# facebookresearch/any4

Measured on AMD Instinct MI355X. Metric: any4 W4A16 GEMM achieved GB/s (m=1, n=k=4096, g=128), higher is better.
Workload: dtype bf16

## Files before the change

any4_amd/csrc/tg_common.cuh:

```cuda
#pragma once
#ifndef GEMV_TRACE
#define GEMV_TRACE 0
#endif
#include <hip/hip_runtime.h>
#include <stdint.h>
#include <stdlib.h>
#include <string.h>
#include <atomic>
#include <type_traits>
#include <utility>

#include "../../include/tinygemm_hip.h"

struct GemmParams {
  const char* x;
  const char* w;
  const char* qinfo;
  const char* lut;
  char* y;
  int32_t m, wrows, k;
  int32_t ntiles;
  int32_t ksuper;
  int32_t gshift;
  int32_t ngroups;
// ... 133 lines not shown
}
inline int pair_b16(int dt, int I, bool qmx, GemmParams& p, int64_t batch, hipStream_t st) {
  return dt == TG_BF16 ? pair_b16_bf16(I, qmx, p, batch, st) : pair_b16_f16(I, qmx, p, batch, st);
}
inline int stream(int dt, bool layout_a, int wpl, bool qmx, const GemmParams& p, int64_t coltiles, int64_t batch, hipStream_t st) {
  return dt == TG_BF16 ? stream_bf16(layout_a, wpl, qmx, p, coltiles, batch, st) : stream_f16(layout_a, wpl, qmx, p, coltiles, batch, st);
}
}

namespace {

typedef __attribute__((ext_vector_type(4))) float f32x4;
typedef __attribute__((ext_vector_type(2))) float f32x2;
typedef __attribute__((ext_vector_type(4))) uint32_t u32x4;
typedef __attribute__((ext_vector_type(2))) uint32_t u32x2;
typedef __attribute__((ext_vector_type(8))) __bf16 bf16x8;
typedef __attribute__((ext_vector_type(2))) __bf16 bf16x2;
typedef __attribute__((ext_vector_type(8))) _Float16 f16x8;
typedef __attribute__((ext_vector_type(2))) _Float16 f16x2;

typedef const __attribute__((address_space(3))) float* lds_cfptr;
typedef __attribute__((address_space(3))) float* lds_fptr;
typedef const __attribute__((address_space(3))) uint16_t* lds_cu16ptr;
typedef const __attribute__((address_space(3))) uint32_t* lds_cu32ptr;
typedef __attribute__((address_space(3))) uint32_t* lds_u32ptr;
typedef const __attribute__((address_space(3))) u32x4* lds_cu32x4ptr;
typedef __attribute__((address_space(3))) u32x4* lds_u32x4ptr;
typedef const __attribute__((address_space(3))) f32x4* lds_cf32x4ptr;
typedef __attribute__((address_space(3))) f32x4* lds_f32x4ptr;

__device__ __forceinline__ float u2f(uint32_t u) { return __builtin_bit_cast(float, u); }
__device__ __forceinline__ uint32_t f2u(float f) { return __builtin_bit_cast(uint32_t, f); }

struct BF16 {
  static __device__ __forceinline__ float to_f32(uint16_t h) { return u2f(((uint32_t)h) << 16); }
  static __device__ __forceinline__ float lo_f32(uint32_t pair) { return u2f(pair << 16); }
  static __device__ __forceinline__ float hi_f32(uint32_t pair) { return u2f(pair & 0xffff0000u); }
  static __device__ __forceinline__ uint32_t pack2(float a, float b) {
    f32x2 v = {a, b};
    return __builtin_bit_cast(uint32_t, __builtin_convertvector(v, bf16x2));
  }
  static __device__ __forceinline__ uint16_t from_f32(float a) { return (uint16_t)(pack2(a, 0.f) & 0xffffu); }
  static __device__ __forceinline__ f32x4 mfma(u32x4 a, u32x4 b, f32x4 c) {
    return __builtin_amdgcn_mfma_f32_16x16x32_bf16(__builtin_bit_cast(bf16x8, a), __builtin_bit_cast(bf16x8, b), c, 0, 0, 0);
  }
};
struct F16 {
  static __device__ __forceinline__ float to_f32(uint16_t h) { return (float)__builtin_bit_cast(_Float16, h); }
  static __device__ __forceinline__ float lo_f32(uint32_t pair) { return to_f32((uint16_t)(pair & 0xffffu)); }
  static __device__ __forceinline__ float hi_f32(uint32_t pair) { return to_f32((uint16_t)(pair >> 16)); }
  static __device__ __forceinline__ uint32_t pack2(float a, float b) {
    f32x2 v = {a, b};
    return __builtin_bit_cast(uint32_t, __builtin_convertvector(v, f16x2));
  }
  static __device__ __forceinline__ uint16_t from_f32(float a) { return (uint16_t)(pack2(a, 0.f) & 0xffffu); }
  static __device__ __forceinline__ f32x4 mfma(u32x4 a, u32x4 b, f32x4 c) {
    return __builtin_amdgcn_mfma_f32_16x16x32_f16(__builtin_bit_cast(f16x8, a), __builtin_bit_cast(f16x8, b), c, 0, 0, 0);
  }
};

__device__ const float kMX4Values[16] = {0.0f,  0.5f,  1.0f,  1.5f,  2.0f,  3.0f,  4.0f,  6.0f,
                                         -0.0f, -0.5f, -1.0f, -1.5f, -2.0f, -3.0f, -4.0f, -6.0f};

template <typename DT>
__device__ __forceinline__ void store_rows4(char* yb, const char* bias, int64_t elem, int rowg, f32x4 acc) {
  u32x2 o = {DT::pack2(acc[0], acc[1]), DT::pack2(acc[2], acc[3])};
  if (bias) {
    const u32x2 bv = *reinterpret_cast<const u32x2*>(bias + (int64_t)rowg * 2);
    o[0] = DT::pack2(DT::lo_f32(o[0]) + DT::lo_f32(bv[0]), DT::hi_f32(o[0]) + DT::hi_f32(bv[0]));
    o[1] = DT::pack2(DT::lo_f32(o[1]) + DT::lo_f32(bv[1]), DT::hi_f32(o[1]) + DT::hi_f32(bv[1]));
  }
  *reinterpret_cast<u32x2*>(yb + elem * 2) = o;
}


__device__ __forceinline__ u32x4 transpose_rows4(u32x4 v) {
  const auto s01 = __builtin_amdgcn_permlane16_swap(v[0], v[1], false, false);
  const auto s23 = __builtin_amdgcn_permlane16_swap(v[2], v[3], false, false);
  const auto t02 = __builtin_amdgcn_permlane32_swap(s01[0], s23[0], false, false);
  const auto t13 = __builtin_amdgcn_permlane32_swap(s01[1], s23[1], false, false);
  return u32x4{t02[0], t13[0], t02[1], t13[1]};
}

struct DeviceScope {
  int prev = -1;
  bool ok = true;
  explicit DeviceScope(int device) {
    if (device < 0) return;
    if (hipGetDevice(&prev) != hipSuccess) { ok = false; return; }
    if (prev != device && hipSetDevice(device) != hipSuccess) ok = false;
    if (prev == device) prev = -1;
  }
  ~DeviceScope() {
    if (prev >= 0) (void)hipSetDevice(prev);
  }
};

inline int launch_status() {
  const hipError_t e = hipGetLastError();
  return e == hipSuccess ? 0 : (int)e;
}

inline bool aligned16(const void* p) { return (reinterpret_cast<uintptr_t>(p) & 15u) == 0; }
inline int64_t cdiv(int64_t a, int64_t b) { return (a + b - 1) / b; }
inline int group_shift(int g) { return g == 32 ? 5 : g == 64 ? 6 : g == 128 ? 7 : 8; }

template <typename D, typename F>
auto assign_if_member(D& d, F f, int) -> decltype(f(d)) { f(d); }
template <typename D, typename F>
void assign_if_member(D&, F, long) {}
template <typename D>
void copy_call(D& d, const GemmParams& p) {
#define TG_COPY(f) assign_if_member(d, [&](auto& t) -> decltype((void)(t.f = p.f)) { t.f = p.f; }, 0)
  TG_COPY(x); TG_COPY(w); TG_COPY(qinfo); TG_COPY(lut); TG_COPY(y);
  TG_COPY(m); TG_COPY(wrows); TG_COPY(k); TG_COPY(ntiles); TG_COPY(ksuper); TG_COPY(gshift); TG_COPY(ngroups); TG_COPY(qtype);
  TG_COPY(stride_x); TG_COPY(stride_w); TG_COPY(stride_qinfo); TG_COPY(stride_lut); TG_COPY(stride_y);
  TG_COPY(bias); TG_COPY(stride_bias); TG_COPY(bias_row_stride);
  TG_COPY(norm_w); TG_COPY(norm_eps); TG_COPY(epilogue); TG_COPY(x_tc); TG_COPY(y_tc); TG_COPY(dry);
#undef TG_COPY
}

template <auto KERN>
int prepare_lds_kernel() {
  static std::atomic<uint64_t> done{0};
  int dev = 0;
  if (hipGetDevice(&dev) != hipSuccess) return TG_E_DEVICE;
  if (dev >= 0 && dev < 64 && ((done.load(std::memory_order_relaxed) >> dev) & 1u)) return 0;
  hipFuncAttributes fa;
  hipError_t e = hipFuncGetAttributes(&fa, reinterpret_cast<const void*>(KERN));
  if (e != hipSuccess) return (int)e;
  if (fa.sharedSizeBytes != 0) return TG_E_INTERNAL;
  e = hipFuncSetAttribute(reinterpret_cast<const void*>(KERN), hipFuncAttributeMaxDynamicSharedMemorySize, 160 * 1024);
  if (e != hipSuccess) return (int)e;
  if (dev >= 0 && dev < 64) done.fetch_or(1ull << dev, std::memory_order_relaxed);
  return 0;
}


inline int cu_count() {
  static std::atomic<int> cache[64];
  int dev = 0;
  if (hipGetDevice(&dev) != hipSuccess || dev < 0 || dev >= 64) return 256;
  int v = cache[dev].load(std::memory_order_relaxed);
  if (v > 0) return v;
  if (hipDeviceGetAttribute(&v, hipDeviceAttributeMultiprocessorCount, dev) != hipSuccess || v <= 0) v = 256;
  cache[dev].store(v, std::memory_order_relaxed);
  return v;
}


#if !defined(TG_DEV) && !defined(TG_DEV_MIN)
#if defined(TG_PAIR_R) || defined(TG_PAIR_ABL) || defined(TG_PAIR_MR1) || defined(TG_PAIR_NSG2) || defined(TG_PAIR_MR1_GPS) || defined(TG_PAIR_RA) ||   \
    defined(TG_PAIR_RA1) || defined(TG_PAIR_RB16) || defined(TG_B16_CHUNK) || defined(TG_PAIR_MIN_ITEMS) || defined(TG_XG_CHUNK) || defined(TG_PAIR_WGS) || \
    defined(TG_PAIR_NSG2_M1) || defined(TG_PAIR_FORCE_XG) || defined(TG_XR_MIN_M) || defined(TG_XR_R) || defined(TG_XR_R8K) || defined(TG_XR_RMX)
#error "the TG_PAIR_* / TG_XG_* / TG_B16_* tuning constants can only be overridden in developer builds (-DTG_DEV or -DTG_DEV_MIN)"
#endif
#endif
#ifndef TG_PAIR_R
#define TG_PAIR_R 2
#endif
#ifndef TG_PAIR_ABL
#define TG_PAIR_ABL 0
#endif
#ifndef TG_PAIR_MR1
#define TG_PAIR_MR1 1
#endif
#ifndef TG_PAIR_NSG2
#define TG_PAIR_NSG2 1
#endif
#ifndef TG_PAIR_NSG2_M1
#define TG_PAIR_NSG2_M1 1
#endif
#ifndef TG_PAIR_MR1_GPS
#define TG_PAIR_MR1_GPS 1
#endif
#ifndef TG_PAIR_RA
#define TG_PAIR_RA 2
#endif
#ifndef TG_PAIR_RA1
#define TG_PAIR_RA1 1
#endif
#ifndef TG_PAIR_RB16
#define TG_PAIR_RB16 2
#endif
#ifndef TG_B16_CHUNK
#define TG_B16_CHUNK 4
#endif
#ifndef TG_TILE_W8_MIN_M
#define TG_TILE_W8_MIN_M 17
#endif
#ifndef TG_TILE_MIN_M_SPLIT
#define TG_TILE_MIN_M_SPLIT 17
#endif
#ifndef TG_TILE_MIN_M
#define TG_TILE_MIN_M 65
#endif
#ifndef TG_M1_DEFAULT_MFMA
#define TG_M1_DEFAULT_MFMA 0
#endif
#ifndef TG_PAIR_MIN_ITEMS
#define TG_PAIR_MIN_ITEMS 192
#endif
#ifndef TG_XG_CHUNK
#define TG_XG_CHUNK 4
#endif
#ifndef TG_XR_MIN_M
#define TG_XR_MIN_M 2
#endif
#ifndef TG_XR_RMX
#define TG_XR_RMX 8
#endif
#ifndef TG_XR_R8K
#define TG_XR_R8K 2
#endif
#ifndef TG_XR_R
#define TG_XR_R 4
#endif
#ifndef TG_PAIR_WGS
#define TG_PAIR_WGS 512
#endif

}
```

any4_amd/csrc/w4_gemm_pair.cuh:

```cuda
#pragma once

__device__ __forceinline__ int64_t tc_a_index(int r, int c, int ctiles) {
  const int t = (r & 7) * 4 + ((c & 7) >> 1);
  const int j = (c & 1) + 2 * ((r >> 3) & 1) + 4 * ((c >> 3) & 1);
  return (((int64_t)(r >> 4) * ctiles + (c >> 4)) * 32 + t) * 8 + j;
}
__device__ __forceinline__ void tc_a_load_chunk(const char* xb, int a, int ch, int ktiles, uint32_t (&d)[16]) {
#pragma unroll
  for (int dw = 0; dw < 16; ++dw) d[dw] = *reinterpret_cast<const uint32_t*>(xb + tc_a_index(a, ch * 32 + 2 * dw, ktiles) * 2);
}

__device__ __forceinline__ u32x4 mx4_cvt_word(uint32_t w, float scale) {
  u32x4 r;
  r[0] = __builtin_bit_cast(uint32_t, __builtin_amdgcn_cvt_scalef32_pk_bf16_fp4(w, scale, 0));
  r[1] = __builtin_bit_cast(uint32_t, __builtin_amdgcn_cvt_scalef32_pk_bf16_fp4(w, scale, 1));
  r[2] = __builtin_bit_cast(uint32_t, __builtin_amdgcn_cvt_scalef32_pk_bf16_fp4(w, scale, 2));
  r[3] = __builtin_bit_cast(uint32_t, __builtin_amdgcn_cvt_scalef32_pk_bf16_fp4(w, scale, 3));
  return r;
}

__device__ __forceinline__ uint32_t mx4_cvt_byte(uint32_t w, float scale, int sel) {
  switch (sel) {
    case 0: return __builtin_bit_cast(uint32_t, __builtin_amdgcn_cvt_scalef32_pk_bf16_fp4(w, scale, 0));
    case 1: return __builtin_bit_cast(uint32_t, __builtin_amdgcn_cvt_scalef32_pk_bf16_fp4(w, scale, 1));
    case 2: return __builtin_bit_cast(uint32_t, __builtin_amdgcn_cvt_scalef32_pk_bf16_fp4(w, scale, 2));
    default: return __builtin_bit_cast(uint32_t, __builtin_amdgcn_cvt_scalef32_pk_bf16_fp4(w, scale, 3));
  }
}

#ifndef TG_PAIR_M1_DOT
#define TG_PAIR_M1_DOT 1
#endif
template <typename DT>
__device__ __forceinline__ float dot2_pair(uint32_t a, uint32_t b, float acc) {
  if constexpr (std::is_same<DT, BF16>::value)
    return __builtin_amdgcn_fdot2_f32_bf16(__builtin_bit_cast(bf16x2, a), __builtin_bit_cast(bf16x2, b), acc, false);
  else
    return __builtin_amdgcn_fdot2(__builtin_bit_cast(f16x2, a), __builtin_bit_cast(f16x2, b), acc, false);
}

struct PairParams {
  const char* x;
  const char* w;
  const char* qinfo;
  const char* lut;
  char* y;
  int32_t m, wrows, k;
  int32_t ntiles;
  int32_t ksuper;
  int32_t gshift;
  int32_t ngroups;
  int32_t qtype;
  int32_t spw;
  int32_t nsg_shift;
  int32_t gch_mask;
  int32_t x_pitch;
  int32_t lds_x;
  int32_t lds_xs;
  int32_t lds_red;
  int32_t rused;
  int32_t xs_rows;
  int32_t red_lanes;
  int32_t red_alias;
  int32_t rblocks;
  int32_t cblocks;
  int32_t items;
  int64_t stride_x, stride_w, stride_qinfo, stride_lut, stride_y;
  const char* bias;
  int64_t stride_bias;
  int64_t bias_row_stride;
  const char* norm_w;
  float norm_eps;
  int32_t epilogue;
  int32_t dry;
  const char* xp;
  const char* xsum;
  int64_t stride_xp, stride_xsum;
  int32_t xw_pitch;
  int32_t xw_bytes;
  int32_t chunk;
  int32_t x_tc, y_tc;
  int32_t y_tiles;
};

typedef __attribute__((ext_vector_type(16))) float f32x16;

template <typename DT>
__device__ __forceinline__ f32x16 mfma32(u32x4 a, u32x4 b, f32x16 c) {
  if constexpr (std::is_same<DT, BF16>::value)
    return __builtin_amdgcn_mfma_f32_32x32x16_bf16(__builtin_bit_cast(bf16x8, a), __builtin_bit_cast(bf16x8, b), c, 0, 0, 0);
  else
    return __builtin_amdgcn_mfma_f32_32x32x16_f16(__builtin_bit_cast(f16x8, a), __builtin_bit_cast(f16x8, b), c, 0, 0, 0);
}

typedef __attribute__((ext_vector_type(4))) float f32x4_t;
template <typename DT>
__device__ __forceinline__ f32x4_t mfma16(u32x4 a, u32x4 b, f32x4_t c) {
  if constexpr (std::is_same<DT, BF16>::value)
    return __builtin_amdgcn_mfma_f32_16x16x32_bf16(__builtin_bit_cast(bf16x8, a), __builtin_bit_cast(bf16x8, b), c, 0, 0, 0);
  else
    return __builtin_amdgcn_mfma_f32_16x16x32_f16(__builtin_bit_cast(f16x8, a), __builtin_bit_cast(f16x8, b), c, 0, 0, 0);
}

__device__ __forceinline__ uint32_t bfi(uint32_t mask, uint32_t a, uint32_t b) {
  uint32_t d;
  asm("v_bfi_b32 %0, %1, %2, %3" : "=v"(d) : "s"(mask), "v"(a), "v"(b));
  return d;
}

template <typename DT>
__device__ __forceinline__ float dot2_ones(uint32_t pair, float acc) {
  if constexpr (std::is_same<DT, BF16>::value)
    return __builtin_amdgcn_fdot2_f32_bf16(__builtin_bit_cast(bf16x2, pair), __builtin_bit_cast(bf16x2, 0x3f803f80u), acc, false);
  else
    return __builtin_amdgcn_fdot2(__builtin_bit_cast(f16x2, pair), __builtin_bit_cast(f16x2, 0x3c003c00u), acc, false);
}

template <typename DT>
__device__ __forceinline__ float chunk_sumsq(const uint32_t (&d)[16]) {
  float s = 0.f;
#pragma unroll
  for (int j = 0; j < 16; ++j) {
    if constexpr (std::is_same<DT, BF16>::value)
      s = __builtin_amdgcn_fdot2_f32_bf16(__builtin_bit_cast(bf16x2, d[j]), __builtin_bit_cast(bf16x2, d[j]), s, false);
    else
      s = __builtin_amdgcn_fdot2(__builtin_bit_cast(f16x2, d[j]), __builtin_bit_cast(f16x2, d[j]), s, false);
  }
  return s;
}
template <typename DT>
__device__ __forceinline__ void chunk_rmsnorm(uint32_t (&d)[16], float rs, const u32x4 (&gw)[4]) {
#pragma unroll
  for (int j = 0; j < 4; ++j) {
    const u32x4 g = gw[j];
#pragma unroll
    for (int e = 0; e < 4; ++e) {
      const uint32_t v = d[4 * j + e];
      const float lo = DT::to_f32(DT::from_f32(DT::lo_f32(v) * rs)) * DT::lo_f32(g[e]);
      const float hi = DT::to_f32(DT::from_f32(DT::hi_f32(v) * rs)) * DT::hi_f32(g[e]);
      d[4 * j + e] = DT::pack2(lo, hi);
    }
  }
}
template <typename DT>
__device__ __forceinline__ uint16_t swiglu16(float gsum, float usum) {
  const float g = DT::to_f32(DT::from_f32(gsum)), u = DT::to_f32(DT::from_f32(usum));
  return DT::from_f32(DT::to_f32(DT::from_f32(g / (1.f + __expf(-g)))) * u);
}

template <typename DT, int I, int GPS, int MR, bool QMX, int R, int NSG = 0, int ABL = 0, bool XG = false, int LAY = 0, bool NORM = false>
__global__ void __launch_bounds__(512, 4) w4_gemm_pair_kernel(const PairParams p) {
  constexpr bool LA = LAY == 1, LB = LAY == 2, T16 = LAY != 0;
  constexpr bool DOT = TG_PAIR_M1_DOT && ABL != 100 && MR == 1 && !T16 && (QMX || NSG > 0);
  constexpr bool MXC = QMX;
  static_assert(!NORM || (!XG && !T16 && !QMX), "fused RMSNorm: the workgroup stages the whole activation block itself");
  constexpr int WAVES = 8;
  constexpr int TILES = 2;
  constexpr int WT = LA ? 1 : TILES;
  constexpr int RW = T16 ? 32 : 32 * TILES;
  static_assert(!T16 || (XG && MR == 4 && (LB || I == 2 || I == 4)), "16x16x32 tiles: workspace activations, one pass of up to 16 rows");
  constexpr int NW = LB ? I / 2 : I;
  using acc_t = typename std::conditional<T16, f32x4_t, f32x16>::type;
  constexpr int CPS = I / 2;
  constexpr int CPG = CPS / GPS;
  constexpr int MREGS = MR == 1 ? 4 : MR;
  constexpr int RF = MR;
  constexpr int MA = T16 ? 16 : 2 * MREGS;
  constexpr int NXW = T16 ? I / 2 : XG ? (MA * 2 * I + 63) / 64 : 1;
  static_assert(!XG || MR <= 4, "XG: one pass is at most 8 activation rows");

  constexpr uint32_t lds0 = 0u;
  const uint32_t lds_x = lds0 + (uint32_t)p.lds_x;
  const uint32_t lds_xs = lds0 + (uint32_t)p.lds_xs;
  const uint32_t lds_red = lds0 + (uint32_t)p.lds_red;

  const int tid = threadIdx.x;
  const int lane = tid & 63;
  const int wave = __builtin_amdgcn_readfirstlane(tid >> 6);
  const int c = lane & 31;
  const int h = lane >> 5;
  const int xa = DOT ? 0 : T16 ? lane & 15 : c;
  const int xq = T16 ? lane >> 4 : 2 * h;
  const int hh = T16 ? lane >> 4 : h;
  auto wrow_local = [&](int t) -> int { return LA ? 16 * ((lane & 15) >> 3) + (lane & 7) + 8 * t : LB ? 16 * t + (lane & 15) : t * 32 + c; };
  const int tcol = tid & 63;
  const int tcol_row = LA ? 16 * ((tcol & 15) >> 3) + (tcol & 7) + 8 * (tcol >> 5) : LB ? 16 * (tcol >> 5) + (tcol & 15) : tcol;

  constexpr bool RR = XG;
  const int chunk = RR ? p.chunk : 1;
  const int it_stride = RR ? (int)gridDim.x * chunk - (chunk - 1) : 1;
  const int it_begin = RR ? (int)blockIdx.x * chunk : (int)(((int64_t)blockIdx.x * p.items) / gridDim.x);
  const int it_end = RR ? p.items : (int)(((int64_t)(blockIdx.x + 1) * p.items) / gridDim.x);
  const int per_problem = p.rblocks * p.cblocks;

  const int s_begin = wave * p.spw;
  const int nl = max(min(p.spw, p.ksuper - s_begin), 0);

  struct Item {
    int b, ct, rb;
  };
  auto decode = [&](int it) -> Item {
    const int b = it / per_problem, r = it - b * per_problem;
    const int ct = r / p.rblocks;
    return Item{b, ct, r - ct * p.rblocks};
  };
  const int adv_b = it_stride / per_problem, adv_r = it_stride - adv_b * per_problem;
  auto advance = [&](const Item& e, bool big) -> Item {
    int b = e.b + (big ? adv_b : 0), r = e.ct * p.rblocks + e.rb + (big ? adv_r : 1);
    if (r >= per_problem) { r -= per_problem; ++b; }
    const int ct = p.cblocks == 1 ? 0 : r / p.rblocks;
    return Item{b, ct, r - ct * p.rblocks};
  };

  uint32_t lp[8];
  auto lut_const = [&]() {
#pragma unroll
    for (int e = 0; e < 16; e += 2) {
      float v0, v1;
      if (p.qtype == TG_Q_INT4) {
        v0 = (float)(e - 8);
        v1 = (float)(e - 7);
      } else {
        const int e1 = e + 1;
        v0 = (e & 8 ? -1.f : 1.f) * ((e & 7) < 5 ? 0.5f * (e & 7) : ((e & 7) == 5 ? 3.f : (e & 7) == 6 ? 4.f : 6.f));
        v1 = (e1 & 8 ? -1.f : 1.f) * ((e1 & 7) < 5 ? 0.5f * (e1 & 7) : ((e1 & 7) == 5 ? 3.f : (e1 & 7) == 6 ? 4.f : 6.f));
      }
      lp[e >> 1] = DT::pack2(v0, v1);
    }
  };
  const bool lut_loaded = p.qtype == TG_Q_ANY4_GLOBAL || p.qtype == TG_Q_ANY4_ROWWISE;
  auto lut_request = [&](const Item& e) {
    const int lrow = min(e.rb * RW + tcol_row, p.wrows - 1);
    const char* lsrc = p.lut + (int64_t)e.b * p.stride_lut + (p.qtype == TG_Q_ANY4_ROWWISE ? (int64_t)lrow * 32 : 0);
    const u32x4 l0 = reinterpret_cast<const u32x4*>(lsrc)[0];
    const u32x4 l1 = reinterpret_cast<const u32x4*>(lsrc)[1];
#pragma unroll
    for (int j = 0; j < 4; ++j) { lp[j] = l0[j]; lp[4 + j] = l1[j]; }
  };

  struct Slot {
    uint32_t w[WT][I];
    uint32_t q[TILES][GPS];
    u32x4 xw[NXW];
  };
  Slot ring[R];
  struct Rows {
    uint32_t wbase[WT];
    uint32_t qrow[TILES];
    uint32_t qrow4[TILES];
    const char* wb;
    const char* qb;
    const char* xpb;
    uint32_t xblk;
    uint32_t xoff[NXW];
  };
  auto rows_of = [&](const Item& e) -> Rows {
    Rows r;
#pragma unroll
    for (int t = 0; t < TILES; ++t) {
      const int row = min(e.rb * RW + wrow_local(t), p.wrows - 1);
      r.qrow[t] = (uint32_t)row;
      r.qrow4[t] = (uint32_t)row * 4u;
      if constexpr (!LA) {
        const int nt = min(row >> 3, p.ntiles - 1);
        r.wbase[t] = ((uint32_t)nt * (uint32_t)p.ksuper * 32u + (uint32_t)(4 * (row & 7) + (LB ? lane >> 4 : 2 * h))) * (uint32_t)(2 * I);
      }
    }
    if constexpr (LA) {
      const int mt = min(e.rb * 2 + ((lane & 15) >> 3), p.ntiles - 1);
      r.wbase[0] = ((uint32_t)mt * (uint32_t)p.ksuper * 32u + (uint32_t)(4 * (lane & 7) + (lane >> 4))) * (uint32_t)(4 * I);
    }
    r.wb = p.w + (int64_t)e.b * p.stride_w;
    r.qb = p.qinfo + (int64_t)e.b * p.stride_qinfo;
    if constexpr (XG) {
      const int rows = min(p.m - e.ct * MA, MA);
      r.xpb = p.xp + (int64_t)e.b * p.stride_xp + (int64_t)e.ct * MA * p.k * 2;
      r.xblk = (uint32_t)(rows * 32 * I);
      if constexpr (T16) {
        r.xblk = (uint32_t)((rows + 1) * 64);
        r.xoff[0] = (uint32_t)(((lane >> 4) * (rows + 1) + min(lane & 15, rows)) * 16);
      } else {
#pragma unroll
        for (int i = 0; i < NXW; ++i) r.xoff[i] = (uint32_t)(lane + 64 * i) * 16u < r.xblk ? (uint32_t)(lane + 64 * i) * 16u : 0u;
      }
    } else {
      r.xpb = nullptr;
      r.xblk = 0;
#pragma unroll
      for (int i = 0; i < NXW; ++i) r.xoff[i] = 0;
    }
    return r;
  };
  auto pin = [](uint32_t& v) -> uint32_t { asm volatile("" : "+v"(v)); return v; };
  auto issue = [&](Rows& rw, int s, Slot& sl, bool valid, bool needq) {
    auto uni = [](uint32_t v) -> uint32_t { return (uint32_t)__builtin_amdgcn_readfirstlane((int)v); };
    const uint32_t sv = valid ? (uint32_t)s : 0u;
    if constexpr (XG) {
#pragma unroll
      for (int i = 0; i < NXW; ++i) {
        if constexpr (T16) {
          if constexpr (ABL == 9 || ABL == 13) sl.xw[i] = u32x4{rw.xoff[0], (uint32_t)s, 0x3f803f80u, 0x3f803f80u};
          else if constexpr (ABL == 12) sl.xw[i] = *reinterpret_cast<const u32x4*>(rw.xpb + uni((uint32_t)i * rw.xblk) + pin(rw.xoff[0]));
          else sl.xw[i] = *reinterpret_cast<const u32x4*>(rw.xpb + uni((sv * CPS + (uint32_t)i) * rw.xblk) + pin(rw.xoff[0]));
          continue;
        }
        if constexpr (ABL == 9) sl.xw[i] = u32x4{rw.xoff[i], (uint32_t)s, 0x3f803f80u, 0x3f803f80u};
// ... 32 lines not shown
      }
    }
  };

  constexpr int EBS = QMX ? 16 / GPS : 1;
  u32x4 ecur[TILES], enext[TILES];
  int eoff_next = 0;
  auto e_request = [&](Rows& rw, int blk, bool valid) {
    const int start = s_begin * GPS + blk * 16;
    const int st = max(min(start & ~3, p.ngroups - 16), 0);
    eoff_next = start - st;
#pragma unroll
    for (int t = 0; t < TILES; ++t)
      enext[t] = *reinterpret_cast<const u32x4*>(rw.qb + (uint32_t)__builtin_amdgcn_readfirstlane(valid ? st : 0) + rw.qrow[t] * (uint32_t)p.ngroups);
  };
  int ebase = 0;
  auto e_dword = [&](int t, int gi) -> uint32_t {
    const int dw = (gi + ebase) >> 2;
    return ecur[t][dw & 3];
  };
  auto e_scale = [&](uint32_t d, int gi) -> float {
    const uint32_t e23 = __builtin_amdgcn_ubfe(d, (uint32_t)(((gi + ebase) & 3) * 8), 8u) << 23;
    const float sc = u2f(e23 > 0x00400000u ? e23 : 0x00400000u);
    return __builtin_fmaf(sc, 0.f, sc);
  };

  const int nch = p.k >> 5;
  auto x_load = [&](const char* xb, int a0, int xi, uint32_t (&d)[16]) {
    const int a = xi / nch, ch = xi - a * nch;
    if (p.x_tc) {
      tc_a_load_chunk(xb, a0 + a, ch, p.k >> 4, d);
      return;
    }
    const u32x4* src = reinterpret_cast<const u32x4*>(xb + ((int64_t)(a0 + a) * p.k + ch * 32) * 2);
#pragma unroll
    for (int j = 0; j < 4; ++j) {
      const u32x4 v = src[j];
      d[4 * j] = v[0]; d[4 * j + 1] = v[1]; d[4 * j + 2] = v[2]; d[4 * j + 3] = v[3];
    }
  };
  auto x_store = [&](int xi, bool on, const uint32_t (&d)[16]) {
    const int a = on ? xi / nch : 0, ch = on ? xi - (xi / nch) * nch : 0;
    if (on) {
      const uint32_t dst = lds_x + (uint32_t)(a * p.x_pitch + ch * 64);
#pragma unroll
      for (int q = 0; q < 4; ++q) {
        u32x4 o;
        o[0] = __builtin_amdgcn_perm(d[q + 4], d[q], 0x05040100u);
        o[1] = __builtin_amdgcn_perm(d[q + 12], d[q + 8], 0x05040100u);
        o[2] = __builtin_amdgcn_perm(d[q + 4], d[q], 0x07060302u);
        o[3] = __builtin_amdgcn_perm(d[q + 12], d[q + 8], 0x07060302u);
        *(lds_u32x4ptr)(dst + (uint32_t)(q * 16)) = o;
      }
    }
    if constexpr (QMX) return;
    float sum = 0.f;
#pragma unroll
    for (int j = 0; j < 16; ++j) sum = dot2_ones<DT>(d[j], sum);
    for (int o = 1; o <= p.gch_mask; o <<= 1) sum += __shfl_xor(sum, o);
    if (on && (ch & p.gch_mask) == 0) *(lds_fptr)(lds_xs + (uint32_t)(((ch >> (p.gshift - 5)) * p.xs_rows + a) * 4)) = sum;
  };
  auto x_stage = [&](int b, int a0, int mrows, bool pre, uint32_t (&xd)[16]) {
    const char* xb = p.x + (int64_t)b * p.stride_x;
    const int xtotal = mrows * nch;
    if constexpr (NORM) {
      const bool on = tid < xtotal;
      if (!pre) {
#pragma unroll
        for (int j = 0; j < 16; ++j) xd[j] = 0u;
        if (on) x_load(xb, a0, tid, xd);
      }
      const int a = on ? tid / nch : 0;
      u32x4 gw[4];
#pragma unroll
      for (int j = 0; j < 4; ++j) gw[j] = reinterpret_cast<const u32x4*>(p.norm_w + (on ? tid - a * nch : 0) * 64)[j];
      float ss = chunk_sumsq<DT>(xd);
      ss = tgl::wave_sum(ss);
      if (lane == 0) *(lds_fptr)(lds_xs + (uint32_t)(wave * 4)) = ss;
      __syncthreads();
      ss = 0.f;
      for (int w0 = a * (nch >> 6); w0 < (a + 1) * (nch >> 6); ++w0) ss += *(lds_fptr)(lds_xs + (uint32_t)(w0 * 4));
      __syncthreads();
      if (on) chunk_rmsnorm<DT>(xd, rsqrtf(ss * (1.0f / (float)p.k) + p.norm_eps), gw);
      pre = true;
    }
    for (int it0 = 0; it0 < xtotal; it0 += 512) {
      const int xi = it0 + tid;
      const bool on = xi < xtotal;
      if (!(pre && it0 == 0)) {
#pragma unroll
        for (int j = 0; j < 16; ++j) xd[j] = 0u;
        if (on) x_load(xb, a0, xi, xd);
      }
      x_store(xi, on, xd);
    }
    if constexpr (!QMX)
      for (int idx = tid; idx < p.ngroups * p.xs_rows; idx += 512)
        if ((idx & (p.xs_rows - 1)) >= mrows) *(lds_fptr)(lds_xs + (uint32_t)(idx * 4)) = 0.f;
    if (tid < CPS * 4) *(lds_u32x4ptr)(lds_x + (uint32_t)(mrows * p.x_pitch + tid * 16)) = u32x4{0, 0, 0, 0};
  };

  constexpr int NXS = T16 ? 2 : 0;
  float xsn[2] = {0.f, 0.f};
  auto xs_request = [&](const Item& e) {
    if constexpr (XG && !QMX) {
      const float* src = reinterpret_cast<const float*>(p.xsum + (int64_t)e.b * p.stride_xsum) + (int64_t)e.ct * p.ngroups * p.xs_rows;
      const int total = p.ngroups * p.xs_rows;
#pragma unroll
      for (int j = 0; j < NXS; ++j) xsn[j] = src[min(tid + 512 * j, total - 1)];
    }
  };
  auto xs_stage = [&](int b, int ct, int mrows) {
    const float* src = reinterpret_cast<const float*>(p.xsum + (int64_t)b * p.stride_xsum) + (int64_t)ct * p.ngroups * p.xs_rows;
    if constexpr (!QMX) {
      const int total = p.ngroups * p.xs_rows;
#pragma unroll
      for (int j = 0; j < NXS; ++j) {
        const int idx = tid + 512 * j;
        if (idx < total) *(lds_fptr)(lds_xs + (uint32_t)(idx * 4)) = (idx & (p.xs_rows - 1)) < mrows ? xsn[j] : 0.f;
      }
      for (int idx = tid + 512 * NXS; idx < total; idx += 512)
        *(lds_fptr)(lds_xs + (uint32_t)(idx * 4)) = (idx & (p.xs_rows - 1)) < mrows ? src[idx] : 0.f;
    }
    if (tid < CPS * 4) *(lds_u32x4ptr)(lds_x + (uint32_t)(WAVES * p.xw_bytes + tid * 16)) = u32x4{0, 0, 0, 0};
  };

  if (it_begin >= it_end) return;
  const Item first = decode(it_begin);
  if (lut_loaded) lut_request(first);
  else lut_const();
  xs_request(first);
  int staged_b = XG ? -1 : first.b, staged_ct = first.ct;
  uint32_t xd0[16];
  if constexpr (!XG) {
    const int mrows0 = min(p.m - first.ct * MA, MA);
#pragma unroll
    for (int j = 0; j < 16; ++j) xd0[j] = 0u;
    if (tid < mrows0 * nch) x_load(p.x + (int64_t)first.b * p.stride_x, first.ct * MA, tid, xd0);
  }
  Rows rcur = rows_of(first);
  if constexpr (QMX) e_request(rcur, 0, nl > 0);
#pragma unroll
  for (int j = 0; j < R; ++j) {
    __builtin_amdgcn_sched_barrier(0);
    issue(rcur, s_begin + j, ring[j], j < nl, NSG == 0 || j % NSG == 0);
  }
  __builtin_amdgcn_sched_barrier(0);
  if constexpr (!XG) x_stage(first.b, first.ct * MA, min(p.m - first.ct * MA, MA), true, xd0);

  uint32_t colreg[TILES];
#pragma unroll
  for (int t = 0; t < TILES; ++t) colreg[t] = (uint32_t)((T16 ? 32 * t + 16 * ((lane >> 4) & 1) + (lane & 15) : t * 32 + c) * 4);

  int table_b = -1;
  Item inext = first;
  int cpos = 0;
  for (int it = it_begin, step = 1; it < it_end; it += step) {
    const bool big = cpos + 1 >= chunk;
    step = big ? it_stride : 1;
    cpos = big ? 0 : cpos + 1;
    const Item cur = inext;
    const int row0 = cur.rb * RW;
    const int a0 = cur.ct * MA;
    const int mrows = min(p.m - a0, MA);
    const bool has_next = it + step < it_end;
    if (has_next) inext = advance(cur, big);
    Rows rnext = rows_of(inext);

    if (!MXC && (it == it_begin || p.qtype == TG_Q_ANY4_ROWWISE || p.red_alias ||
        (p.qtype == TG_Q_ANY4_GLOBAL && cur.b != table_b))) {
      table_b = cur.b;
      uint32_t hw = lp[0];
#pragma unroll
      for (int j = 1; j < 8; ++j) hw = (wave == j) ? lp[j] : hw;
      const uint32_t base = lds0 + (uint32_t)(wave * 2 * 16 * 256 + tcol * 4);
#pragma unroll
      for (int a = 0; a < 16; ++a) {
        const uint32_t e0 = __builtin_amdgcn_perm(hw, lp[a >> 1], (a & 1) ? 0x05040302u : 0x05040100u);
        const uint32_t e1 = __builtin_amdgcn_perm(hw, lp[a >> 1], (a & 1) ? 0x07060302u : 0x07060100u);
        const lds_u32ptr tb = (lds_u32ptr)base;
        tb[a * 64] = e0;
        tb[(16 + a) * 64] = e1;
      }
    }
    if (cur.b != staged_b || cur.ct != staged_ct) {
      staged_b = cur.b;
      staged_ct = cur.ct;
      if constexpr (XG) {
        if (ABL != 11) xs_stage(cur.b, cur.ct, mrows);
      } else {
        uint32_t xd[16];
        x_stage(cur.b, a0, mrows, false, xd);
      }
    }
    if (lut_loaded) lut_request(inext);
    xs_request(inext);
    __syncthreads();

    const bool a_on = xa < mrows;
    const uint32_t xzero = XG ? lds_x + (uint32_t)(WAVES * p.xw_bytes) : lds_x + (uint32_t)(mrows * p.x_pitch);
    const uint32_t xs_mask = 4 * hh < p.xs_rows ? 0xffffffffu : 0u;
    const uint32_t xs_lane = 4 * hh < p.xs_rows ? lds_xs + (uint32_t)(4 * hh * 4) : xzero;
    const uint32_t xwbuf = lds_x + (uint32_t)(wave * p.xw_bytes);
    const uint32_t xrow = !a_on ? xzero : XG ? xwbuf + (uint32_t)(xa * p.xw_pitch + xq * 16) : lds_x + (uint32_t)(xa * p.x_pitch + xq * 16);
    const uint32_t xmask = a_on && !XG ? 0xffffffffu : 0u;
    const uint32_t xw_dst = xwbuf + (uint32_t)((lane / (2 * I)) * p.xw_pitch + (lane % (2 * I)) * 16);

    acc_t acc[TILES];
    float yacc[TILES][RF];
#pragma unroll
    for (int t = 0; t < TILES; ++t) {
#pragma unroll
      for (int r = 0; r < (T16 ? 4 : 16); ++r) acc[t][r] = 0.f;
#pragma unroll
      for (int r = 0; r < RF; ++r) yacc[t][r] = 0.f;
    }
    float gs[TILES], gz[TILES];
    float xsv[RF];
#pragma unroll
    for (int t = 0; t < TILES; ++t) gs[t] = gz[t] = 0.f;
#pragma unroll
    for (int r = 0; r < RF; ++r) xsv[r] = 0.f;

    auto unpack_q = [&](uint32_t q, float& s, float& z) {
      if constexpr (QMX) {
        s = u2f(q == 255u ? 0x7fc00000u : (q == 0u ? 0x00400000u : (q << 23)));
        z = 0.f;
      } else {
        s = DT::lo_f32(q);
        z = DOT && h ? 0.f : DT::hi_f32(q);
      }
    };
    constexpr bool DIFF = MR == 1;
    float dacc[TILES] = {0.f, 0.f};
    float prev[TILES][RF];
#pragma unroll
    for (int t = 0; t < TILES; ++t)
#pragma unroll
      for (int r = 0; r < RF; ++r) prev[t][r] = 0.f;
    auto finalize = [&]() {
#pragma unroll
      for (int t = 0; t < TILES; ++t) {
        if constexpr (DOT) {
          const float d = dacc[t] - prev[t][0];
          prev[t][0] = dacc[t];
          yacc[t][0] = __builtin_fmaf(gz[t], xsv[0], __builtin_fmaf(gs[t], d, yacc[t][0]));
          continue;
        }
        if constexpr (DIFF && RF == 1 && !QMX) {
          float a0 = acc[t][0];
          asm volatile("" : "+v"(a0));
          float d;
          asm("v_sub_f32 %0, %1, %2" : "=v"(d) : "v"(a0), "v"(prev[t][0]));
          prev[t][0] = a0;
          asm("v_fmac_f32 %0, %1, %2" : "+v"(yacc[t][0]) : "v"(gs[t]), "v"(d));
          asm("v_fmac_f32 %0, %1, %2" : "+v"(yacc[t][0]) : "v"(gz[t]), "v"(xsv[0]));
          asm volatile("" : "+v"(acc[t]));
          asm volatile("" ::"v"(acc[t][1]), "v"(acc[t][2]), "v"(acc[t][3]));
          continue;
        }
#pragma unroll
        for (int r = 0; r < RF; ++r) {
          float d = acc[t][r];
          if constexpr (DIFF) {
            d -= prev[t][r];
            prev[t][r] = acc[t][r];
          }
          yacc[t][r] = __builtin_fmaf(gs[t], d, yacc[t][r]);
          if constexpr (!QMX) yacc[t][r] = __builtin_fmaf(gz[t], xsv[r], yacc[t][r]);
        }
        if constexpr (DIFF) asm volatile("" : "+v"(acc[t]));
        if constexpr (RF == 1) asm volatile("" ::"v"(acc[t][1]), "v"(acc[t][2]), "v"(acc[t][3]));
      }
    };
    bool pending = false;
    acc_t zero16;
#pragma unroll
    for (int r = 0; r < (T16 ? 4 : 16); ++r) zero16[r] = 0.f;
    uint32_t edw[TILES] = {0u, 0u};
    auto consume = [&](int s, const Slot& sl, int j_slot) {
      const uint32_t xst = xrow + ((uint32_t)(s * CPS * 64) & xmask);
      if constexpr (XG && !T16) {
#pragma unroll
        for (int i = 0; i < NXW; ++i)
          if constexpr (ABL != 10) *(lds_u32x4ptr)(xw_dst + (uint32_t)(i * (64 / (2 * I)) * p.xw_pitch)) = sl.xw[i];
      }
      if constexpr (ABL == 6) {
#pragma unroll
        for (int t = 0; t < WT; ++t)
#pragma unroll
          for (int j = 0; j < I; ++j) acc[t][0] += u2f(sl.w[t][j]);
        acc[0][1] += u2f(sl.q[0][0] ^ sl.q[1][0]);
        return;
      }
#pragma unroll
      for (int u = 0; u < (T16 ? CPS : 2 * CPS); ++u) {
        const int jc = T16 ? u : u >> 1, qq = T16 ? 0 : u & 1;
        const bool qfirst = T16 || qq == 0, qlast = T16 || qq == 1;
        const int chunk = s * CPS + jc;
        constexpr bool STATIC_G = GPS > 1 || NSG > 0;
        const int gpos = NSG > 0 ? j_slot % NSG : 0;
        const bool gfirst = qfirst && (GPS > 1 ? jc % CPG == 0 : NSG > 0 ? (gpos == 0 && jc == 0) : (chunk & p.gch_mask) == 0);
        const bool glast = qlast && (GPS > 1 ? jc % CPG == CPG - 1 : NSG > 0 ? (gpos == NSG - 1 && jc == CPS - 1) : (chunk & p.gch_mask) == p.gch_mask);
        u32x4 xf;
        u32x4 bf[TILES];
        if constexpr (ABL == 5) xf = u32x4{xrow, (uint32_t)s, (uint32_t)jc, (uint32_t)qq};
        else if constexpr (T16) xf = sl.xw[jc];
        else xf = *(lds_cu32x4ptr)(xst + (uint32_t)(jc * 64 + 16 * qq));
#pragma unroll
        for (int t = 0; t < TILES; ++t) {
          if constexpr (MXC) {
            if (gfirst) {
              const int gg0 = GPS == 1 ? 0 : jc / CPG;
              const int gi = (s - s_begin) * GPS + gg0;
              if (gg0 == 0) edw[t] = e_dword(t, gi);
              gs[t] = e_scale(edw[t], gi);
            }
          }
          if constexpr (LA) {
            uint32_t uw[2];
#pragma unroll
            for (int e = 0; e < 2; ++e) {
              const uint32_t w = sl.w[0][2 * jc + e];
              uw[e] = t == 0 ? bfi(0x0f0f0f0fu, w, w >> 4) : bfi(0xf0f0f0f0u, w, w << 4);
            }
#pragma unroll
            for (int j = 0; j < 4; ++j) {
              if constexpr (MXC) {
                bf[t][j] = mx4_cvt_byte(uw[j & 1], gs[t], t + 2 * (j >> 1));
                continue;
              }
              const uint32_t addr = __builtin_amdgcn_perm(uw[j & 1], colreg[t], 0x0c0c0400u + ((uint32_t)(t + 2 * (j >> 1)) << 8));
              if constexpr (ABL == 1) bf[t][j] = addr;
              else bf[t][j] = *(lds_cu32ptr)(addr);
            }
          } else if constexpr (LB) {
            const uint32_t w = sl.w[t][jc];
            if constexpr (MXC) {
              bf[t] = mx4_cvt_word(w, gs[t]);
            } else {
#pragma unroll
              for (int j = 0; j < 4; ++j) {
                const uint32_t addr = __builtin_amdgcn_perm(w, colreg[t], 0x0c0c0400u + ((uint32_t)j << 8));
                if constexpr (ABL == 1) bf[t][j] = addr;
                else bf[t][j] = *(lds_cu32ptr)(addr);
              }
            }
          } else if constexpr (MXC) {
            bf[t] = mx4_cvt_word(sl.w[t][qq * CPS + jc], gs[t]);
          } else {
            const uint32_t w = sl.w[t < WT ? t : 0][qq * CPS + jc];
#pragma unroll
            for (int j = 0; j < 4; ++j) {
              const uint32_t addr = __builtin_amdgcn_perm(w, colreg[t], 0x0c0c0400u + ((uint32_t)j << 8));
              if constexpr (ABL == 1) bf[t][j] = addr;
              else bf[t][j] = *(lds_cu32ptr)(addr);
            }
          }
        }
        if constexpr (MXC) {
        } else if constexpr (STATIC_G) {
          if (gfirst) finalize();
        } else if (qfirst && pending) {
          finalize();
          pending = false;
        }
        __builtin_amdgcn_sched_barrier(0);
        if (ABL != 7 && gfirst && !MXC) {
          const int gg = GPS == 1 ? 0 : jc / CPG;
#pragma unroll
          for (int t = 0; t < TILES; ++t) {
            if constexpr (QMX) {
              const int gi = (s - s_begin) * GPS + gg;
              if (gg == 0) edw[t] = e_dword(t, gi);
              gs[t] = e_scale(edw[t], gi);
            } else {
              unpack_q(sl.q[t][gg], gs[t], gz[t]);
            }
          }
          if constexpr (!QMX) {
            const uint32_t xsa = xs_lane + ((uint32_t)((((chunk * 32) >> p.gshift) * p.xs_rows) * 4) & xs_mask);
            if constexpr (RF == 1) {
              xsv[0] = *(const __attribute__((address_space(3))) float*)(lds_xs + (uint32_t)((((chunk * 32) >> p.gshift) * p.xs_rows) * 4));
            } else {
#pragma unroll
              for (int r4 = 0; r4 < MREGS / 4; ++r4) {
                const f32x4 vv = *(lds_cf32x4ptr)(xsa + ((uint32_t)(r4 * 32) & xs_mask));
                xsv[4 * r4] = vv[0]; xsv[4 * r4 + 1] = vv[1]; xsv[4 * r4 + 2] = vv[2]; xsv[4 * r4 + 3] = vv[3];
              }
            }
          }
        }
#pragma unroll
        for (int t = 0; t < TILES; ++t) {
          if constexpr (DOT) {
#pragma unroll
            for (int j = 0; j < 4; ++j) dacc[t] = dot2_pair<DT>(bf[t][j], xf[j], dacc[t]);
          } else
          if constexpr (ABL == 4) acc[t][0] += u2f(bf[t][0] ^ bf[t][1] ^ bf[t][2] ^ bf[t][3] ^ xf[0] ^ xf[1] ^ xf[2] ^ xf[3]);
          else if constexpr (T16) acc[t] = mfma16<DT>(xf, bf[t], (ABL != 7 && gfirst && !MXC) ? zero16 : acc[t]);
          else if (ABL != 7 && !DIFF && gfirst && !MXC) acc[t] = mfma32<DT>(xf, bf[t], zero16);
          else acc[t] = mfma32<DT>(xf, bf[t], acc[t]);
        }
        if constexpr (STATIC_G && !DOT) {
#pragma unroll
          for (int t = 0; t < TILES; ++t) asm volatile("" : "+v"(acc[t]));
        }
        if (ABL != 7 && !STATIC_G && glast && !MXC) pending = true;
        __builtin_amdgcn_sched_barrier(0);
      }
    };

    const int rounds = max((nl + R - 1) / R, 1);
    int l0 = 0;
    const int nblk = QMX ? max((nl + EBS - 1) / EBS, 1) : 1;
    for (int blk = 0; blk < nblk; ++blk) {
      const bool lastb = blk + 1 == nblk;
      if constexpr (QMX) {
#pragma unroll
        for (int t = 0; t < TILES; ++t) ecur[t] = enext[t];
        ebase = eoff_next - blk * 16;
        e_request(lastb ? rnext : rcur, lastb ? 0 : blk + 1, lastb ? has_next && nl > 0 : true);
      }
      const int rend = lastb ? rounds - 1 : (blk + 1) * (EBS / R);
      for (int rd = l0 / R; rd < rend; ++rd, l0 += R) {
#pragma unroll
        for (int j = 0; j < R; ++j) {
          consume(s_begin + l0 + j, ring[j], j);
          issue(rcur, s_begin + l0 + j + R, ring[j], l0 + j + R < nl, NSG == 0 || j % NSG == 0);
        }
      }
    }
#pragma unroll
    for (int j = 0; j < R; ++j) {
      if (l0 + j < nl) consume(s_begin + l0 + j, ring[j], j);
      issue(rnext, s_begin + j, ring[j], has_next && j < nl, NSG == 0 || j % NSG == 0);
    }
    if constexpr (MXC) {
#pragma unroll
      for (int t = 0; t < TILES; ++t)
#pragma unroll
        for (int r = 0; r < RF; ++r) yacc[t][r] = DOT ? dacc[t] : acc[t][r];
    } else if (pending || GPS > 1 || NSG > 0) finalize();
    if constexpr (DOT) {
#pragma unroll
      for (int t = 0; t < TILES; ++t) yacc[t][0] += __shfl_xor(yacc[t][0], 32);
    }
    if constexpr (ABL == 6) yacc[0][0] += acc[0][0] + acc[0][1] + acc[1][0];
    if constexpr (ABL == 7) { yacc[0][0] = acc[0][0]; yacc[1][0] = acc[1][0]; }

    if (p.red_alias) __syncthreads();
#pragma unroll
    for (int t = 0; t < TILES; ++t) {
#pragma unroll
      for (int r = 0; r < RF; ++r)
        if (r < p.rused && lane < p.red_lanes)
          *(lds_fptr)(lds_red + (uint32_t)((((wave * TILES + t) * p.rused + r) * p.red_lanes + lane) * 4)) = yacc[t][r];
    }
    __syncthreads();
    {
      char* yb = p.y + (int64_t)cur.b * p.stride_y;
      static_assert(TILES == 2, "the output index split below assumes two tiles");
      const int rl_shift = p.red_lanes == 64 ? 6 : 5;
      for (int o = tid; o < TILES * p.rused * p.red_lanes; o += 512) {
        const int l = o & (p.red_lanes - 1), q = o >> rl_shift;
        const int t = q >= p.rused ? 1 : 0, r = q - t * p.rused;
        const int a = T16 ? r + 4 * (l >> 4) : (r & 3) + 8 * (r >> 2) + 4 * (l >> 5);
        const int row = row0 + (LA ? 16 * ((l & 15) >> 3) + (l & 7) + 8 * t : LB ? 16 * t + (l & 15) : t * 32 + (l & 31));
        if (a < mrows && row < p.wrows) {
          float sum = 0.f;
#pragma unroll
          for (int w = 0; w < WAVES; ++w) sum += *(lds_fptr)(lds_red + (uint32_t)((((w * TILES + t) * p.rused + r) * p.red_lanes + l) * 4));
          if (!T16 && p.epilogue == TG_EPI_SWIGLU) {
            if ((l & 15) < 8) {
              float up = 0.f;
#pragma unroll
              for (int w = 0; w < WAVES; ++w) up += *(lds_fptr)(lds_red + (uint32_t)((((w * TILES + t) * p.rused + r) * p.red_lanes + l + 8) * 4));
              *reinterpret_cast<uint16_t*>(yb + ((int64_t)(a0 + a) * (p.wrows >> 1) + ((row >> 4) << 3) + (row & 7)) * 2) = swiglu16<DT>(sum, up);
            }
            continue;
          }
          uint16_t o16 = DT::from_f32(sum);
          if (p.bias)
            o16 = DT::from_f32(DT::lo_f32(o16) + DT::lo_f32(*reinterpret_cast<const uint16_t*>(p.bias + (int64_t)cur.b * p.stride_bias + ((int64_t)(a0 + a) * p.bias_row_stride + row) * 2)));
          *reinterpret_cast<uint16_t*>(yb + (p.y_tc ? tc_a_index(a0 + a, row, p.y_tiles) : (int64_t)(a0 + a) * p.wrows + row) * 2) = o16;
        }
      }
    }
    if (p.red_alias) __syncthreads();
    rcur = rnext;
  }
}

struct XPrepParams {
  const char* x;
  char* xp;
  char* xsum;
  int32_t m, k, ma, cps, gshift, gch_mask, ngroups, xs_rows;
  int32_t la;
  int32_t x_tc;
  int64_t stride_x, stride_xp, stride_xsum;
};

template <typename DT>
__global__ void __launch_bounds__(256) w4_xprep_kernel(const XPrepParams p) {
  const int nch = p.k >> 5;
  const int xi = blockIdx.x * 256 + threadIdx.x;
  const bool on = xi < p.m * nch;
  const int a = on ? xi / nch : 0, ch = on ? xi - a * nch : 0;
  const int b = blockIdx.y;
  uint32_t d[16];
#pragma unroll
  for (int j = 0; j < 16; ++j) d[j] = 0u;
  if (on && p.x_tc) {
    tc_a_load_chunk(p.x + (int64_t)b * p.stride_x, a, ch, p.k >> 4, d);
  } else if (on) {
    const u32x4* src = reinterpret_cast<const u32x4*>(p.x + (int64_t)b * p.stride_x + ((int64_t)a * p.k + ch * 32) * 2);
#pragma unroll
    for (int j = 0; j < 4; ++j) {
      const u32x4 v = src[j];
      d[4 * j] = v[0]; d[4 * j + 1] = v[1]; d[4 * j + 2] = v[2]; d[4 * j + 3] = v[3];
    }
  }
  const int ct = a / p.ma, ar = a - ct * p.ma;
  const int rows = min(p.m - ct * p.ma, p.ma);
  if (on) {
    const int s = ch / p.cps, jc = ch - s * p.cps;
    char* dst = p.xp + (int64_t)b * p.stride_xp + (int64_t)ct * p.ma * p.k * 2 +
                (p.la ? ((int64_t)ch * 4 * (rows + 1) + ar) * 16 : ((int64_t)(s * rows + ar) * p.cps + jc) * 64);
    const int qstride = p.la ? rows + 1 : 1;
#pragma unroll
    for (int q = 0; q < 4; ++q) {
      u32x4 o;
      o[0] = __builtin_amdgcn_perm(d[q + 4], d[q], 0x05040100u);
      o[1] = __builtin_amdgcn_perm(d[q + 12], d[q + 8], 0x05040100u);
      o[2] = __builtin_amdgcn_perm(d[q + 4], d[q], 0x07060302u);
      o[3] = __builtin_amdgcn_perm(d[q + 12], d[q + 8], 0x07060302u);
      reinterpret_cast<u32x4*>(dst)[q * qstride] = o;
    }
    if (p.la && ar == 0)
#pragma unroll
      for (int q = 0; q < 4; ++q) reinterpret_cast<u32x4*>(dst)[q * qstride + rows] = u32x4{0, 0, 0, 0};
  }
  float sum = 0.f;
#pragma unroll
  for (int j = 0; j < 16; ++j) sum = dot2_ones<DT>(d[j], sum);
  for (int o = 1; o <= p.gch_mask; o <<= 1) sum += __shfl_xor(sum, o);
  if (on && (ch & p.gch_mask) == 0)
    reinterpret_cast<float*>(p.xsum + (int64_t)b * p.stride_xsum)[((int64_t)ct * p.ngroups + (ch >> (p.gshift - 5))) * p.xs_rows + ar] = sum;
}
```

Measured before the change: 6630.

## Broadcast activations via DPP dot2c and keep early-round x in registers for m=1

For the m=1 dot-product path with I==4, each lane now loads a single activation dword from LDS. The dot uses v_dot2c_*_dpp with row_newbcast to broadcast the right lane's activation, replacing a 16-byte LDS vector load per step. When activations are not quantized-MX, the first few rounds' activation dwords are also loaded into registers once per staged tile and reused. The change adds inline asm with manual s_nop hazard padding and a large switch over broadcast lanes, plus a dev script that scans the compiled assembly for DPP hazards. It risks extra instructions, register pressure and hazard-related stalls.

```diff
diff --git a/any4_amd/csrc/tg_common.cuh b/any4_amd/csrc/tg_common.cuh
--- a/any4_amd/csrc/tg_common.cuh
+++ b/any4_amd/csrc/tg_common.cuh
@@ -309,7 +309,8 @@
 #if !defined(TG_DEV) && !defined(TG_DEV_MIN)
 #if defined(TG_PAIR_R) || defined(TG_PAIR_ABL) || defined(TG_PAIR_MR1) || defined(TG_PAIR_NSG2) || defined(TG_PAIR_MR1_GPS) || defined(TG_PAIR_RA) ||   \
     defined(TG_PAIR_RA1) || defined(TG_PAIR_RB16) || defined(TG_B16_CHUNK) || defined(TG_PAIR_MIN_ITEMS) || defined(TG_XG_CHUNK) || defined(TG_PAIR_WGS) || \
-    defined(TG_PAIR_NSG2_M1) || defined(TG_PAIR_FORCE_XG) || defined(TG_XR_MIN_M) || defined(TG_XR_R) || defined(TG_XR_R8K) || defined(TG_XR_RMX)
+    defined(TG_PAIR_NSG2_M1) || defined(TG_PAIR_FORCE_XG) || defined(TG_XR_MIN_M) || defined(TG_XR_R) || defined(TG_XR_R8K) || defined(TG_XR_RMX) || \
+    defined(TG_PAIR_M1_XDPP)
 #error "the TG_PAIR_* / TG_XG_* / TG_B16_* tuning constants can only be overridden in developer builds (-DTG_DEV or -DTG_DEV_MIN)"
 #endif
 #endif
@@ -319,6 +320,9 @@
 #ifndef TG_PAIR_ABL
 #define TG_PAIR_ABL 0
 #endif
+#ifndef TG_PAIR_M1_XDPP
+#define TG_PAIR_M1_XDPP 2
+#endif
 #ifndef TG_PAIR_MR1
 #define TG_PAIR_MR1 1
 #endif
diff --git a/any4_amd/csrc/w4_gemm_pair.cuh b/any4_amd/csrc/w4_gemm_pair.cuh
--- a/any4_amd/csrc/w4_gemm_pair.cuh
+++ b/any4_amd/csrc/w4_gemm_pair.cuh
@@ -37,6 +37,26 @@
     return __builtin_amdgcn_fdot2_f32_bf16(__builtin_bit_cast(bf16x2, a), __builtin_bit_cast(bf16x2, b), acc, false);
   else
     return __builtin_amdgcn_fdot2(__builtin_bit_cast(f16x2, a), __builtin_bit_cast(f16x2, b), acc, false);
+}
+
+template <typename DT, int N>
+__device__ __forceinline__ float dot2c_bcast(uint32_t x, uint32_t b, float acc) {
+  static_assert(N >= 0 && N < 16, "row_newbcast takes a lane of the 16-lane row");
+  if constexpr (std::is_same<DT, BF16>::value)
+    asm("v_dot2c_f32_bf16_dpp %0, %1, %2 row_newbcast:%3 row_mask:0xf bank_mask:0xf" : "+v"(acc) : "v"(x), "v"(b), "n"(N));
+  else
+    asm("v_dot2c_f32_f16_dpp %0, %1, %2 row_newbcast:%3 row_mask:0xf bank_mask:0xf" : "+v"(acc) : "v"(x), "v"(b), "n"(N));
+  return acc;
+}
+template <typename DT>
+__device__ __forceinline__ float dot2c_bcast_sel(int n, uint32_t x, uint32_t b, float acc) {
+  switch (n) {
+#define TG_BC(N_) case N_: return dot2c_bcast<DT, N_>(x, b, acc);
+    TG_BC(0) TG_BC(1) TG_BC(2) TG_BC(3) TG_BC(4) TG_BC(5) TG_BC(6) TG_BC(7)
+    TG_BC(8) TG_BC(9) TG_BC(10) TG_BC(11) TG_BC(12) TG_BC(13) TG_BC(14)
+#undef TG_BC
+    default: return dot2c_bcast<DT, 15>(x, b, acc);
+  }
 }
 
 struct PairParams {
@@ -152,6 +172,7 @@
 __global__ void __launch_bounds__(512, 4) w4_gemm_pair_kernel(const PairParams p) {
   constexpr bool LA = LAY == 1, LB = LAY == 2, T16 = LAY != 0;
   constexpr bool DOT = TG_PAIR_M1_DOT && ABL != 100 && MR == 1 && !T16 && (QMX || NSG > 0);
+  constexpr int XDPP = (DOT && I == 4 && !XG && ABL != 5) ? TG_PAIR_M1_XDPP : 0;
   constexpr bool MXC = QMX;
   static_assert(!NORM || (!XG && !T16 && !QMX), "fused RMSNorm: the workgroup stages the whole activation block itself");
   constexpr int WAVES = 8;
@@ -490,6 +511,14 @@
 #pragma unroll
   for (int t = 0; t < TILES; ++t) colreg[t] = (uint32_t)((T16 ? 32 * t + 16 * ((lane >> 4) & 1) + (lane & 15) : t * 32 + c) * 4);
 
+  const uint32_t xdl = lds_x + (uint32_t)(((lane >> 3) & 1) * 64 + (2 * h + ((lane >> 2) & 1)) * 16 + (lane & 3) * 4);
+  auto x_bcast = [&](int s) -> uint32_t {
+    return *(lds_cu32ptr)(xdl + (uint32_t)(s * CPS * 64));
+  };
+  constexpr bool XRES = XDPP == 2 && !QMX;
+  constexpr int XRR = !XRES ? 0 : R <= 2 ? 3 : 1;
+  uint32_t xres[XRR * R + 1];
+  bool xres_stale = true;
   int table_b = -1;
   Item inext = first;
   int cpos = 0;
@@ -524,6 +553,7 @@
     if (cur.b != staged_b || cur.ct != staged_ct) {
       staged_b = cur.b;
       staged_ct = cur.ct;
+      xres_stale = true;
       if constexpr (XG) {
         if (ABL != 11) xs_stage(cur.b, cur.ct, mrows);
       } else {
@@ -534,6 +564,13 @@
     if (lut_loaded) lut_request(inext);
     xs_request(inext);
     __syncthreads();
+    if constexpr (XRES) {
+      if (xres_stale) {
+#pragma unroll
+        for (int i = 0; i < XRR * R; ++i) xres[i] = x_bcast(i < nl ? s_begin + i : 0);
+        xres_stale = false;
+      }
+    }
 
     const bool a_on = xa < mrows;
     const uint32_t xzero = XG ? lds_x + (uint32_t)(WAVES * p.xw_bytes) : lds_x + (uint32_t)(mrows * p.x_pitch);
@@ -616,7 +653,7 @@
 #pragma unroll
     for (int r = 0; r < (T16 ? 4 : 16); ++r) zero16[r] = 0.f;
     uint32_t edw[TILES] = {0u, 0u};
-    auto consume = [&](int s, const Slot& sl, int j_slot) {
+    auto consume = [&](int s, const Slot& sl, int j_slot, uint32_t xd) {
       const uint32_t xst = xrow + ((uint32_t)(s * CPS * 64) & xmask);
       if constexpr (XG && !T16) {
 #pragma unroll
@@ -644,7 +681,7 @@
         u32x4 bf[TILES];
         if constexpr (ABL == 5) xf = u32x4{xrow, (uint32_t)s, (uint32_t)jc, (uint32_t)qq};
         else if constexpr (T16) xf = sl.xw[jc];
-        else xf = *(lds_cu32x4ptr)(xst + (uint32_t)(jc * 64 + 16 * qq));
+        else if constexpr (XDPP == 0) xf = *(lds_cu32x4ptr)(xst + (uint32_t)(jc * 64 + 16 * qq));
 #pragma unroll
         for (int t = 0; t < TILES; ++t) {
           if constexpr (MXC) {
@@ -733,7 +770,10 @@
         for (int t = 0; t < TILES; ++t) {
           if constexpr (DOT) {
 #pragma unroll
-            for (int j = 0; j < 4; ++j) dacc[t] = dot2_pair<DT>(bf[t][j], xf[j], dacc[t]);
+            for (int j = 0; j < 4; ++j) {
+              if constexpr (XDPP != 0) dacc[t] = dot2c_bcast_sel<DT>(4 * u + j, xd, bf[t][j], dacc[t]);
+              else dacc[t] = dot2_pair<DT>(bf[t][j], xf[j], dacc[t]);
+            }
           } else
           if constexpr (ABL == 4) acc[t][0] += u2f(bf[t][0] ^ bf[t][1] ^ bf[t][2] ^ bf[t][3] ^ xf[0] ^ xf[1] ^ xf[2] ^ xf[3]);
           else if constexpr (T16) acc[t] = mfma16<DT>(xf, bf[t], (ABL != 7 && gfirst && !MXC) ? zero16 : acc[t]);
@@ -747,11 +787,25 @@
         if (ABL != 7 && !STATIC_G && glast && !MXC) pending = true;
         __builtin_amdgcn_sched_barrier(0);
       }
+      if constexpr (XDPP != 0) asm volatile("s_nop 3" : "+v"(dacc[0]), "+v"(dacc[1]));
     };
 
     const int rounds = max((nl + R - 1) / R, 1);
     int l0 = 0;
     const int nblk = QMX ? max((nl + EBS - 1) / EBS, 1) : 1;
+    if constexpr (XRES) {
+#pragma unroll
+      for (int rr = 0; rr < XRR; ++rr) {
+        if (rr < rounds - 1) {
+#pragma unroll
+          for (int j = 0; j < R; ++j) {
+            consume(s_begin + rr * R + j, ring[j], j, xres[rr * R + j]);
+            issue(rcur, s_begin + rr * R + j + R, ring[j], rr * R + j + R < nl, NSG == 0 || j % NSG == 0);
+          }
+          l0 = (rr + 1) * R;
+        }
+      }
+    }
     for (int blk = 0; blk < nblk; ++blk) {
       const bool lastb = blk + 1 == nblk;
       if constexpr (QMX) {
@@ -762,16 +816,19 @@
       }
       const int rend = lastb ? rounds - 1 : (blk + 1) * (EBS / R);
       for (int rd = l0 / R; rd < rend; ++rd, l0 += R) {
+        uint32_t xdp[R];
+#pragma unroll
+        for (int j = 0; j < R; ++j) xdp[j] = XDPP != 0 ? x_bcast(s_begin + l0 + j) : 0u;
 #pragma unroll
         for (int j = 0; j < R; ++j) {
-          consume(s_begin + l0 + j, ring[j], j);
+          consume(s_begin + l0 + j, ring[j], j, xdp[j]);
           issue(rcur, s_begin + l0 + j + R, ring[j], l0 + j + R < nl, NSG == 0 || j % NSG == 0);
         }
       }
     }
 #pragma unroll
     for (int j = 0; j < R; ++j) {
-      if (l0 + j < nl) consume(s_begin + l0 + j, ring[j], j);
+      if (l0 + j < nl) consume(s_begin + l0 + j, ring[j], j, XDPP != 0 ? x_bcast(s_begin + l0 + j) : 0u);
       issue(rnext, s_begin + j, ring[j], has_next && j < nl, NSG == 0 || j % NSG == 0);
     }
     if constexpr (MXC) {
diff --git a/dev/dpp_hazards.py b/dev/dpp_hazards.py
--- /dev/null
+++ b/dev/dpp_hazards.py
@@ -0,0 +1,80 @@
+import importlib.util
+import os
+import re
+import subprocess
+import sys
+import tempfile
+
+ROOT = os.path.join(os.path.dirname(os.path.abspath(__file__)), "..")
+spec = importlib.util.spec_from_file_location("_build", os.path.join(ROOT, "any4_amd", "build.py"))
+b = importlib.util.module_from_spec(spec)
+spec.loader.exec_module(b)
+
+
+def regs(text):
+    out = set()
+    for lo, hi in re.findall(r"v\[(\d+):(\d+)\]", text):
+        out.update(range(int(lo), int(hi) + 1))
+    out.update(int(r) for r in re.findall(r"\bv(\d+)\b", text))
+    return out
+
+
+def scan(path):
+    ins = [s for s in (l.strip() for l in open(path)) if s and not s.startswith((";", ".", "//")) and not re.match(r"^[\w.$]+:", s)]
+    found, n = [], 0
+    for i, l in enumerate(ins):
+        m = re.match(r"(v_dot2c_f32_\w+_dpp) v(\d+), v(\d+), v\d+", l)
+        if not m:
+            continue
+        n += 1
+        op, dst, src = m.group(1), int(m.group(2)), int(m.group(3))
+        for back in (1, 2):
+            p = ins[i - back]
+            if p.startswith("v_") and "dot2c" not in p and src in regs(p.split(",")[0]):
+                found.append(f"vector write of a DPP source: {p} | {l}")
+        for back in range(1, 6):
+            p = ins[i - back]
+            if re.search(r"\bexec\b", p.split(",")[0]) or p.startswith(("v_cmpx", "s_and_saveexec", "s_or_saveexec")):
+                found.append(f"EXEC write in front of a DPP instruction: {p} | {l}")
+        ws, j = 0, i + 1
+        while ws < 4 and j < len(ins):
+            p = ins[j]
+            if p.startswith(("s_cbranch", "s_branch", "s_endpgm", "s_setpc")):
+                found.append(f"branch within 4 wait states of a dot result: {l} | {p}")
+                break
+            nop = re.match(r"s_nop (\d+)", p)
+            if nop:
+                ws += int(nop.group(1)) + 1
+            else:
+                if not p.startswith(op) and " " in p and dst in regs(p.split(None, 1)[1]):
+                    if ws < (4 if dst in regs(p.split(",")[0]) else 3):
+                        found.append(f"dot result used after {ws} wait states: {l} | {p}")
+                ws += 1
+            j += 1
+    return n, found
+
+
+if __name__ == "__main__":
+    args = sys.argv[1:]
+    extra = []
+    if "--" in args:
+        extra, args = args[args.index("--") + 1:], args[:args.index("--")]
+    unit = args[0] if args else "tg_pair.hip"
+    bad = 0
+    with tempfile.TemporaryDirectory() as tmp:
+        jobs = []
+        for name, src, defs in b.UNITS:
+            if src == unit:
+                out = os.path.join(tmp, name + ".s")
+                jobs.append((name, out, subprocess.Popen([b.hipcc(), *b.FLAGS, *defs, *extra, "-S", "--cuda-device-only", os.path.join(b.CSRC, src), "-o", out],
+                                                         stderr=subprocess.PIPE, text=True)))
+        for name, out, proc in jobs:
+            err = proc.communicate()[1]
+            if proc.returncode != 0:
+                sys.exit(f"{name}: hipcc failed\n{err}")
+            n, found = scan(out)
+            for f in found:
+                print(f"{name}: {f}")
+            print(f"{name}: {n} DPP dot products, {len(found)} findings")
+            bad += len(found)
+    sys.exit(1 if bad else 0)
```

Measured after the change: 6691, median of 6. No clear change (+0.9%).
